# zhvng/open-musiclm

Measured on NVIDIA H100. Metric: coarse-stage training tokens/sec (positions fed to the transformer per optimiser step / step time), higher is better.
Workload: dtype bf16 (fp16 operands for the forward GEMMs on LayerNorm outputs x weights; fp32 accumulate)

## Files before the change

open-musiclm_b200/csrc/common.cuh:

```cuda
#pragma once
#include <cuda_runtime.h>
#include <cuda_bf16.h>
#include <cuda_fp16.h>
#include <cuda.h>
#include <stdint.h>
#include <stdio.h>

namespace omlm {

void set_last_error(const char* fmt, ...);
#define OMLM_CHECK_ARG(cond, ...)          \
  do {                                     \
    if (!(cond)) {                         \
      ::omlm::set_last_error(__VA_ARGS__); \
      return 1;                            \
    }                                      \
  } while (0)
#define OMLM_CUDA(expr)                                                                       \
  do {                                                                                        \
    cudaError_t _e = (expr);                                                                  \
    if (_e != cudaSuccess) {                                                                  \
      ::omlm::set_last_error("%s:%d %s -> %s", __FILE__, __LINE__, #expr, cudaGetErrorString(_e)); \
      return 1000 + static_cast<int>(_e);                                                     \
    }                                                                                         \
  } while (0)
#define OMLM_LAUNCH_CHECK() OMLM_CUDA(cudaGetLastError())

int make_tmap_bf16_2d(CUtensorMap* out, const void* gptr, uint64_t dim0, uint64_t dim1,
                      uint64_t pitch_bytes, uint32_t box0, uint32_t box1);

int make_tmap_2d(CUtensorMap* out, int elem_bytes, const void* gptr, uint64_t dim0, uint64_t dim1, uint64_t pitch_bytes,
                 uint32_t box0, uint32_t box1);

int make_tmap_bf16_3d(CUtensorMap* out, const void* gptr, uint64_t dim0, uint64_t dim1, uint64_t dim2,
                      uint64_t pitch1_bytes, uint64_t pitch2_bytes, uint32_t box0, uint32_t box1);

int num_sms();

template <typename... KArgs, typename... Args>
inline cudaError_t launch_k(void (*kern)(KArgs...), dim3 grid, dim3 block, size_t smem, cudaStream_t stream, Args&&... args) {
  cudaLaunchConfig_t cfg = {};
  cfg.gridDim = grid; cfg.blockDim = block; cfg.dynamicSmemBytes = smem; cfg.stream = stream;
  return cudaLaunchKernelEx(&cfg, kern, static_cast<KArgs>(args)...);
}
#define OMLM_KLAUNCH(kern, grid, block, smem, stream, ...)                                                   \
  do {                                                                                                       \
    cudaError_t _le = ::omlm::launch_k(kern, dim3(grid), dim3(block), smem, stream, __VA_ARGS__);            \
    if (_le != cudaSuccess) {                                                                                \
      ::omlm::set_last_error("%s:%d launch of %s -> %s", __FILE__, __LINE__, #kern, cudaGetErrorString(_le)); \
      return 1000 + static_cast<int>(_le);                                                                   \
    }                                                                                                        \
  } while (0)

__device__ __forceinline__ float warp_sum(float v) {
#pragma unroll
  for (int o = 16; o > 0; o >>= 1) v += __shfl_xor_sync(0xffffffffu, v, o);
  return v;
}
__device__ __forceinline__ float warp_max(float v) {
#pragma unroll
  for (int o = 16; o > 0; o >>= 1) v = fmaxf(v, __shfl_xor_sync(0xffffffffu, v, o));
  return v;
}
__device__ __forceinline__ uint32_t pack_bf16x2(float lo, float hi) {
  __nv_bfloat162 t = __floats2bfloat162_rn(lo, hi);
  return *reinterpret_cast<uint32_t*>(&t);
}
__device__ __forceinline__ float2 unpack_bf16x2(uint32_t v) {
  __nv_bfloat162 t = *reinterpret_cast<__nv_bfloat162*>(&v);
  return __bfloat1622float2(t);
}
__device__ __forceinline__ float bf16_round(float x) {
  return __bfloat162float(__float2bfloat16_rn(x));
}
enum : int { kFmtBF16 = 0, kFmtF32 = 1, kFmtF16 = 2 };
__device__ __forceinline__ uint32_t pack_f16x2(float lo, float hi) {
  uint32_t r;
  asm("cvt.rn.satfinite.f16x2.f32 %0, %1, %2;" : "=r"(r) : "f"(hi), "f"(lo));
  return r;
}
__device__ __forceinline__ float2 unpack_f16x2(uint32_t v) {
  __half2 t = *reinterpret_cast<__half2*>(&v);
  return __half22float2(t);
}
template <bool F16>
__device__ __forceinline__ uint32_t pack16x2(float lo, float hi) {
  if constexpr (F16) return pack_f16x2(lo, hi); else return pack_bf16x2(lo, hi);
}
template <bool F16>
__device__ __forceinline__ float2 unpack16x2(uint32_t v) {
  if constexpr (F16) return unpack_f16x2(v); else return unpack_bf16x2(v);
}

__device__ __forceinline__ float2 fma2(float2 a, float2 b, float2 c) { return make_float2(fmaf(a.x, b.x, c.x), fmaf(a.y, b.y, c.y)); }
__device__ __forceinline__ float2 mul2(float2 a, float2 b) { return make_float2(__fmul_rn(a.x, b.x), __fmul_rn(a.y, b.y)); }
__device__ __forceinline__ float2 add2(float2 a, float2 b) { return make_float2(__fadd_rn(a.x, b.x), __fadd_rn(a.y, b.y)); }
__device__ __forceinline__ float2 splat2(float v) { return make_float2(v, v); }
__device__ __forceinline__ float rcp_approx(float x) {
  float r;
  asm("rcp.approx.ftz.f32 %0, %1;" : "=f"(r) : "f"(x));
  return r;
}
__device__ __forceinline__ float ex2_approx(float x) {
  float r;
  asm("ex2.approx.ftz.f32 %0, %1;" : "=f"(r) : "f"(x));
// ... 52 lines not shown
```

open-musiclm_b200/csrc/gemm_ffn_up.cu:

```cuda
#include "common.cuh"
#include "ptx.cuh"
#include "../../include/omlm_b200.h"

namespace omlm {

constexpr int kFuBM = 128, kFuBN = 256, kFuBK = 64, kFuStages = 3, kFuRowsOut = 126;
constexpr int kFuA = kFuBM * kFuBK * 2, kFuB = kFuBN * kFuBK * 2, kFuStage = kFuA + kFuB;
constexpr int kFuUPitch = 528;
constexpr int kFuOffU = kFuStages * kFuStage;
constexpr int kFuOffBar = kFuOffU + kFuBM * kFuUPitch;
constexpr int kFuSmem = kFuOffBar + 256 + 1024;
constexpr int kFuThreads = 384;

template <bool F16>
__global__ void __launch_bounds__(kFuThreads, 1)
gemm_ffn_up_kernel(const __grid_constant__ CUtensorMap tmA, const __grid_constant__ CUtensorMap tmB,
                   __nv_bfloat16* __restrict__ u_out, __nv_bfloat16* __restrict__ h_out, float* __restrict__ rowsum,
                   const float* __restrict__ conv_w, int M, int Nseq, int K, int Fp) {
  extern __shared__ __align__(1024) uint8_t smem_raw[];
  uint8_t* smem = smem_raw + ((1024u - (smem_u32(smem_raw) & 1023u)) & 1023u);
  uint64_t* full_bar = reinterpret_cast<uint64_t*>(smem + kFuOffBar);
  uint64_t* empty_bar = full_bar + kFuStages;
  uint8_t* usm = smem + kFuOffU;

  const int wg = threadIdx.x >> 7, lane = threadIdx.x & 31;
  const int m_tiles = (M + kFuRowsOut - 1) / kFuRowsOut;
  const int n_tiles = (2 * Fp) / kFuBN;
  const int kb_total = (K + kFuBK - 1) / kFuBK;
  const int work_total = m_tiles * n_tiles;

  if (threadIdx.x == 0) {
    tma_prefetch_desc(&tmA); tma_prefetch_desc(&tmB);
    for (int i = 0; i < kFuStages; ++i) { mbar_init(&full_bar[i], 1); mbar_init(&empty_bar[i], 2); }
    fence_barrier_init();
  }
  __syncthreads();

  if (wg == 0) {
    asm volatile("setmaxnreg.dec.sync.aligned.u32 40;");
    if (threadIdx.x == 0) {
      int stage = 0; uint32_t phase = 0;
      for (int w = blockIdx.x; w < work_total; w += gridDim.x) {
        const int n_blk = w % n_tiles, m_blk = w / n_tiles;
        for (int kb = 0; kb < kb_total; ++kb) {
          mbar_wait(&empty_bar[stage], phase ^ 1);
          uint8_t* sa = smem + stage * kFuStage;
          mbar_expect_tx(&full_bar[stage], kFuStage);
          tma_load_2d(sa, &tmA, &full_bar[stage], kb * kFuBK, m_blk * kFuRowsOut - 2);
          tma_load_2d(sa + kFuA, &tmB, &full_bar[stage], kb * kFuBK, n_blk * kFuBN);
          if (++stage == kFuStages) { stage = 0; phase ^= 1; }
        }
      }
    }
  } else {
    asm volatile("setmaxnreg.inc.sync.aligned.u32 232;");
    const int cw = wg - 1;
    const int wq = (threadIdx.x >> 5) & 3, qr = lane >> 2, qc = lane & 3;
    const bool leader = (threadIdx.x & 127) == 0;
    const int et = threadIdx.x - 128;
    int stage = 0; uint32_t phase = 0;
    bool first = true;
    for (int w = blockIdx.x; w < work_total; w += gridDim.x) {
      const int n_blk = w % n_tiles, m_blk = w / n_tiles;
      float acc[kFuBN / 2];
#pragma unroll
      for (int i = 0; i < kFuBN / 2; ++i) acc[i] = 0.f;
      int prev = -1;
      for (int kb = 0; kb < kb_total; ++kb) {
        mbar_wait(&full_bar[stage], phase);
        const uint32_t sa = smem_u32(smem + stage * kFuStage) + cw * 8192, sb = smem_u32(smem + stage * kFuStage + kFuA);
        wgmma_fence();
#pragma unroll
        for (int k = 0; k < kFuBK / 16; ++k)
          Wgmma<kFuBN, F16>::template ss<0, 0>(acc, make_smem_desc(sa + k * 32, 16, 1024), make_smem_desc(sb + k * 32, 16, 1024),
                                               (kb > 0 || k > 0) ? 1u : 0u);
        wgmma_commit();
        wgmma_wait<1>();
        if (prev >= 0 && leader) mbar_arrive(&empty_bar[prev]);
        prev = stage;
        if (++stage == kFuStages) { stage = 0; phase ^= 1; }
      }
      wgmma_wait<0>();
      wgmma_reg_fence(acc);
      if (prev >= 0 && leader) mbar_arrive(&empty_bar[prev]);
      float2 wv[3][2], wg2[3][2];
      {
        const float4* wp = reinterpret_cast<const float4*>(conv_w + static_cast<long>(n_blk * kFuBN + lane * 4) * 3);
        const float4* gp = reinterpret_cast<const float4*>(conv_w + static_cast<long>(n_blk * kFuBN + 128 + lane * 4) * 3);
        const float4 a0 = __ldg(wp), a1 = __ldg(wp + 1), a2 = __ldg(wp + 2);
        const float4 b0 = __ldg(gp), b1 = __ldg(gp + 1), b2 = __ldg(gp + 2);
        const float fa[12] = {a0.x, a0.y, a0.z, a0.w, a1.x, a1.y, a1.z, a1.w, a2.x, a2.y, a2.z, a2.w};
        const float fb[12] = {b0.x, b0.y, b0.z, b0.w, b1.x, b1.y, b1.z, b1.w, b2.x, b2.y, b2.z, b2.w};
#pragma unroll
        for (int k = 0; k < 3; ++k)
#pragma unroll
          for (int q = 0; q < 2; ++q) {
            wv[k][q] = make_float2(fa[(2 * q) * 3 + k], fa[(2 * q + 1) * 3 + k]);
            wg2[k][q] = make_float2(fb[(2 * q) * 3 + k], fb[(2 * q + 1) * 3 + k]);
          }
      }
      if (!first) asm volatile("bar.sync 2, 256;" ::: "memory");
      first = false;
#pragma unroll
      for (int hr = 0; hr < 2; ++hr) {
        uint8_t* urow = usm + (cw * 64 + wq * 16 + qr + hr * 8) * kFuUPitch + qc * 4;
#pragma unroll
        for (int i = 0; i < kFuBN / 8; ++i)
          *reinterpret_cast<uint32_t*>(urow + i * 16) = pack16x2<F16>(acc[4 * i + 2 * hr], acc[4 * i + 2 * hr + 1]);
      }
      asm volatile("bar.sync 2, 256;" ::: "memory");
      {
        const int ew = et >> 5;
        const int t0 = 2 + ew * 16;
        const long grow0 = static_cast<long>(m_blk) * kFuRowsOut - 2 + t0;
        const int nrows = min(min(16, kFuBM - t0), static_cast<int>(min(static_cast<long>(16), M - grow0)));
        int pos = static_cast<int>(grow0 % Nseq);
        const uint8_t* rp = usm + t0 * kFuUPitch;
        float2 xv1[2], xg1[2], xv2[2], xg2[2];
        {
          const uint2 a = *reinterpret_cast<const uint2*>(rp - kFuUPitch + lane * 8);
          const uint2 g = *reinterpret_cast<const uint2*>(rp - kFuUPitch + 256 + lane * 8);
          xv1[0] = unpack16x2<F16>(a.x); xv1[1] = unpack16x2<F16>(a.y); xg1[0] = unpack16x2<F16>(g.x); xg1[1] = unpack16x2<F16>(g.y);
        }
        {
          const uint2 a = *reinterpret_cast<const uint2*>(rp - 2 * kFuUPitch + lane * 8);
          const uint2 g = *reinterpret_cast<const uint2*>(rp - 2 * kFuUPitch + 256 + lane * 8);
          xv2[0] = unpack16x2<F16>(a.x); xv2[1] = unpack16x2<F16>(a.y); xg2[0] = unpack16x2<F16>(g.x); xg2[1] = unpack16x2<F16>(g.y);
        }
        if (pos == 1) { xv2[0] = xv2[1] = xg2[0] = xg2[1] = make_float2(0.f, 0.f); }
        float st[32];
        __nv_bfloat16* ug = u_out + grow0 * (2L * Fp) + n_blk * kFuBN + lane * 8;
        __nv_bfloat16* hg = h_out + grow0 * static_cast<long>(Fp) + n_blk * 128 + lane * 4;
#pragma unroll
        for (int r = 0; r < 16; ++r) {
          float s1 = 0.f, s2 = 0.f;
          if (r < nrows) {
            const uint8_t* rr = rp + r * kFuUPitch;
            *reinterpret_cast<uint4*>(ug + static_cast<long>(r) * (2L * Fp)) = *reinterpret_cast<const uint4*>(rr + lane * 16);
            const uint2 a = *reinterpret_cast<const uint2*>(rr + lane * 8);
            const uint2 g = *reinterpret_cast<const uint2*>(rr + 256 + lane * 8);
            const float2 xv0[2] = {unpack16x2<F16>(a.x), unpack16x2<F16>(a.y)}, xg0[2] = {unpack16x2<F16>(g.x), unpack16x2<F16>(g.y)};
            if (pos == 0) {
              const float2 z = make_float2(0.f, 0.f);
              xv1[0] = xv1[1] = xg1[0] = xg1[1] = z;
              xv2[0] = xv2[1] = xg2[0] = xg2[1] = z;
            }
            float2 h[2], sq = make_float2(0.f, 0.f), sm = sq;
#pragma unroll
            for (int q = 0; q < 2; ++q) {
              const float2 yv = fma2(wv[0][q], xv2[q], fma2(wv[1][q], xv1[q], mul2(wv[2][q], xv0[q])));
              const float2 yg = fma2(wg2[0][q], xg2[q], fma2(wg2[1][q], xg1[q], mul2(wg2[2][q], xg0[q])));
              h[q] = mul2(gelu_erf2(yg), yv);
              sm = add2(sm, h[q]);
              sq = fma2(h[q], h[q], sq);
              xv2[q] = xv1[q]; xv1[q] = xv0[q];
              xg2[q] = xg1[q]; xg1[q] = xg0[q];
            }
            s1 = sm.x + sm.y; s2 = sq.x + sq.y;
            *reinterpret_cast<uint2*>(hg + static_cast<long>(r) * Fp) = make_uint2(pack16x2<F16>(h[0].x, h[0].y), pack16x2<F16>(h[1].x, h[1].y));
            if (++pos == Nseq) pos = 0;
          }
          st[2 * r] = s1;
          st[2 * r + 1] = s2;
        }
#pragma unroll
        for (int off = 16; off >= 1; off >>= 1) {
          const bool hi = (lane & off) != 0;
#pragma unroll
          for (int i = 0; i < off; ++i) {
            const float send = hi ? st[i] : st[i + off];
            const float keep = hi ? st[i + off] : st[i];
            st[i] = keep + __shfl_xor_sync(0xffffffffu, send, off);
          }
        }
        if ((lane >> 1) < nrows) rowsum[(grow0 + (lane >> 1)) * (2L * n_tiles) + 2 * n_blk + (lane & 1)] = st[0];
      }
    }
  }
}

}

extern "C" int omlm_gemm_ffn_up(const void* xn, const void* w1_packed, const float* conv_w_packed, void* u_out, void* h_out,
                                float* rowsum, int M, int Nseq, int K, int Fp, int act_f16, int max_ctas, void* stream) {
  using namespace omlm;
  OMLM_CHECK_ARG(M > 0 && Nseq > 0 && K > 0 && K % 8 == 0 && Fp > 0 && Fp % 128 == 0, "gemm_ffn_up: bad shape M=%d K=%d Fp=%d", M, K, Fp);
  CUtensorMap tmA, tmB;
  int rc = make_tmap_bf16_2d(&tmA, xn, static_cast<uint64_t>(K), static_cast<uint64_t>(M), static_cast<uint64_t>(K) * 2, 64, kFuBM);
  if (rc) return rc;
  rc = make_tmap_bf16_2d(&tmB, w1_packed, static_cast<uint64_t>(K), static_cast<uint64_t>(2 * Fp), static_cast<uint64_t>(K) * 2, 64, kFuBN);
  if (rc) return rc;
  static bool configured = false;
  if (!configured) {
    OMLM_CUDA(cudaFuncSetAttribute(gemm_ffn_up_kernel<false>, cudaFuncAttributeMaxDynamicSharedMemorySize, kFuSmem));
    OMLM_CUDA(cudaFuncSetAttribute(gemm_ffn_up_kernel<true>, cudaFuncAttributeMaxDynamicSharedMemorySize, kFuSmem));
    configured = true;
  }
  const int m_tiles = (M + kFuRowsOut - 1) / kFuRowsOut, n_tiles = (2 * Fp) / kFuBN;
  int grid = num_sms();
  if (max_ctas > 0 && max_ctas < grid) grid = max_ctas;
  if (m_tiles * n_tiles < grid) grid = m_tiles * n_tiles;
  auto kern = act_f16 ? gemm_ffn_up_kernel<true> : gemm_ffn_up_kernel<false>;
  OMLM_KLAUNCH((kern), grid, kFuThreads, kFuSmem, reinterpret_cast<cudaStream_t>(stream), 
      tmA, tmB, reinterpret_cast<__nv_bfloat16*>(u_out), reinterpret_cast<__nv_bfloat16*>(h_out), rowsum, conv_w_packed, M,
      Nseq, K, Fp);
  OMLM_LAUNCH_CHECK();
  return 0;
}
```

open-musiclm_b200/csrc/gemm_tc.cu:

```cuda
#include "common.cuh"
#include "ptx.cuh"
#include "../../include/omlm_b200.h"
#include <stdlib.h>
#include <string.h>
#include <algorithm>

namespace omlm {

constexpr int BM = 128;
constexpr int BK = 64;
constexpr int kGemmThreads = 384;

struct EpiParams {
  void* out;
  const float* addend;
  long ldo;
  long ldadd;
  float alpha;
  int out_f32;
  int atomic;
  long split_stride;
  int vec_ok;
  int staged;
  int row_split;
  int row_valid;
  int n_valid;
  const float* rs_gamma;
  const uint8_t* rs_keep;
  float2* rs_part;
  float rs_keep_scale;
  int rs_parts;
};

__device__ __forceinline__ float bf16lo(uint32_t v) { return __uint_as_float(v << 16); }
__device__ __forceinline__ float bf16hi(uint32_t v) { return __uint_as_float(v & 0xffff0000u); }

template <int BN>
struct GemmSmem {
  static constexpr int kABytes = BM * BK * 2;
  static constexpr int kBBytes = BN * BK * 2;
  static constexpr int kStageBytes = kABytes + kBBytes;
  static constexpr int kMaxStages = 8;
};

constexpr int kEpiBoxes = 4;
constexpr int kBoxBytes = 64 * 128;
constexpr int kStagingBytes = 2 * kEpiBoxes * kBoxBytes;

__device__ __forceinline__ void wg_bar_sync(int cw) { asm volatile("bar.sync %0, 128;" ::"r"(1 + cw) : "memory"); }

template <bool F32>
__device__ __forceinline__ uint32_t box_offset(int r, int g, int qc) {
  const int chunk = F32 ? 2 * g + (qc >> 1) : g;
  return r * 128 + ((chunk ^ (r & 7)) << 4) + (F32 ? 8 * (qc & 1) : 4 * qc);
}

__device__ __forceinline__ void load_box(const CUtensorMap* tm, uint8_t* box, uint64_t* bar, int col, int row) {
  mbar_expect_tx(bar, kBoxBytes);
  tma_load_2d(box, tm, bar, col, row);
}

template <int BN, bool RS, bool F32>
__device__ __forceinline__ void epilogue_staged(float (&acc)[BN / 2], const EpiParams& ep, const CUtensorMap* tmO,
                                                const CUtensorMap* tmE, uint8_t* ring, uint64_t* ebar, uint32_t& seq,
                                                uint32_t& ephase, int live, int n_blk, int row0, int M, int N, int cw,
                                                bool leader) {
  constexpr int kCols = F32 ? 32 : 64, kGroups = kCols / 8, kBoxesPerTile = BN / kCols;
  constexpr int kBatch = RS ? 4 : kGroups;
  const bool with_e = RS || ep.addend != nullptr;
  const int lane = threadIdx.x & 31, wq = (threadIdx.x >> 5) & 3, qr = lane >> 2, qc = lane & 3;
  float rs1[2][2] = {{0.f, 0.f}, {0.f, 0.f}}, rs2[2][2] = {{0.f, 0.f}, {0.f, 0.f}};
#pragma unroll
  for (int b = 0; b < kBoxesPerTile; ++b) {
    if (b >= live) break;
    const uint32_t slot = seq % kEpiBoxes;
    uint8_t* box = ring + slot * kBoxBytes;
    if (with_e) {
      mbar_wait(&ebar[slot], (ephase >> slot) & 1u);
      ephase ^= 1u << slot;
    } else {
      if (leader) tma_store_wait_read<kEpiBoxes - 1>();
      wg_bar_sync(cw);
    }
#pragma unroll
    for (int g0 = 0; g0 < kGroups; g0 += kBatch) {
      float2 gam[kBatch];
      uint32_t keep[2][kBatch];
      if constexpr (RS) {
#pragma unroll
        for (int j = 0; j < kBatch; ++j) {
          const int col = n_blk * BN + b * kCols + 8 * (g0 + j) + 2 * qc;
          gam[j] = __ldg(reinterpret_cast<const float2*>(ep.rs_gamma + col));
#pragma unroll
          for (int hr = 0; hr < 2; ++hr) {
            const int row = row0 + wq * 16 + qr + hr * 8;
            keep[hr][j] = (row < M && ep.rs_keep != nullptr) ? ep.rs_keep[static_cast<long>(row) * (N >> 3) + (col >> 3)] : 0xffu;
          }
        }
      }
#pragma unroll
      for (int j = 0; j < kBatch; ++j) {
        const int i = b * kGroups + g0 + j;
#pragma unroll
        for (int hr = 0; hr < 2; ++hr) {
          const int r = wq * 16 + qr + hr * 8;
          uint8_t* p = box + box_offset<F32>(r, g0 + j, qc);
          float v0 = __fmul_rn(acc[4 * i + 2 * hr], ep.alpha), v1 = __fmul_rn(acc[4 * i + 2 * hr + 1], ep.alpha);
          if constexpr (RS) {
            const uint32_t kb = keep[hr][j], hv = *reinterpret_cast<const uint32_t*>(p);
            const int col = n_blk * BN + 8 * i + 2 * qc;
            const int hf = (8 * i) / (BN / 2);
            rs1[hr][hf] = fmaf(gam[j].x, ((kb >> (col & 7)) & 1u) ? v0 : 0.f, rs1[hr][hf]);
            rs1[hr][hf] = fmaf(gam[j].y, ((kb >> ((col + 1) & 7)) & 1u) ? v1 : 0.f, rs1[hr][hf]);
            rs2[hr][hf] = fmaf(v0, bf16lo(hv), rs2[hr][hf]);
            rs2[hr][hf] = fmaf(v1, bf16hi(hv), rs2[hr][hf]);
          }
          if constexpr (F32) {
            if (ep.addend != nullptr) { const float2 a = *reinterpret_cast<const float2*>(p); v0 += a.x; v1 += a.y; }
            *reinterpret_cast<float2*>(p) = make_float2(v0, v1);
          } else {
            *reinterpret_cast<uint32_t*>(p) = pack_bf16x2(v0, v1);
          }
        }
      }
    }
    fence_proxy_async();
    wg_bar_sync(cw);
    if (leader) {
      tma_store_2d(tmO, box, n_blk * BN + b * kCols, row0);
      tma_store_commit();
      if (with_e && b >= 1 && b - 1 + kEpiBoxes < live) {
        const uint32_t s = (seq - 1) % kEpiBoxes;
        tma_store_wait_read<1>();
        load_box(tmE, ring + s * kBoxBytes, &ebar[s], n_blk * BN + (b - 1 + kEpiBoxes) * kCols, row0);
      }
    }
    ++seq;
  }
  if constexpr (RS) {
#pragma unroll
    for (int hr = 0; hr < 2; ++hr)
#pragma unroll
      for (int hf = 0; hf < 2; ++hf) {
        float a1 = rs1[hr][hf], a2 = rs2[hr][hf];
        a1 += __shfl_xor_sync(0xffffffffu, a1, 1); a1 += __shfl_xor_sync(0xffffffffu, a1, 2);
        a2 += __shfl_xor_sync(0xffffffffu, a2, 1); a2 += __shfl_xor_sync(0xffffffffu, a2, 2);
        const int row = row0 + wq * 16 + qr + hr * 8;
        if (qc == 0 && row < M) ep.rs_part[static_cast<long>(row) * ep.rs_parts + 2 * n_blk + hf] = make_float2(a1 * ep.rs_keep_scale, a2);
      }
  }
}

template <int BN, int A_MN, int B_MN, bool F16, bool RS = false>
__global__ void __launch_bounds__(kGemmThreads, 1)
gemm_bf16_kernel(const __grid_constant__ CUtensorMap tmA, const __grid_constant__ CUtensorMap tmB,
                 const __grid_constant__ CUtensorMap tmO, const __grid_constant__ CUtensorMap tmE,
                 const EpiParams ep, const int M, const int N, const int K, const int splits, const int kStages) {
  using S = GemmSmem<BN>;
  extern __shared__ uint8_t smem_raw[];
  uint8_t* smem = smem_raw + ((1024u - (smem_u32(smem_raw) & 1023u)) & 1023u);
  uint8_t* staging = smem + kStages * S::kStageBytes;
  uint64_t* full_bar = reinterpret_cast<uint64_t*>(staging + (ep.staged ? kStagingBytes : 0));
  uint64_t* empty_bar = full_bar + S::kMaxStages;
  uint64_t* epi_bar = empty_bar + S::kMaxStages;

  const int wg = threadIdx.x >> 7;
  const int lane = threadIdx.x & 31;

  const int m_tiles = (M + BM - 1) / BM;
  const int n_tiles = (N + BN - 1) / BN;
  const int kb_total = (K + BK - 1) / BK;
  const int kb_per_split = (kb_total + splits - 1) / splits;
  const int tiles_total = m_tiles * n_tiles;
  const int work_total = tiles_total * splits;

  if (threadIdx.x == 0) {
    tma_prefetch_desc(&tmA);
    tma_prefetch_desc(&tmB);
    for (int i = 0; i < kStages; ++i) {
      mbar_init(&full_bar[i], 1);
      mbar_init(&empty_bar[i], 2);
    }
    if (ep.staged) {
      tma_prefetch_desc(&tmO);
      for (int i = 0; i < 2 * kEpiBoxes; ++i) mbar_init(&epi_bar[i], 1);
    }
    fence_barrier_init();
  }
  __syncthreads();

  if (wg == 0) {
    asm volatile("setmaxnreg.dec.sync.aligned.u32 40;");
    if (threadIdx.x == 0) {
      int stage = 0;
      uint32_t phase = 0;
      for (int w = blockIdx.x; w < work_total; w += gridDim.x) {
        const int split = w / tiles_total;
        const int tile = w - split * tiles_total;
        const int n_blk = tile % n_tiles, m_blk = tile / n_tiles;
        const int kb0 = split * kb_per_split;
        const int kb1 = min(kb_total, kb0 + kb_per_split);
        for (int kb = kb0; kb < kb1; ++kb) {
          mbar_wait(&empty_bar[stage], phase ^ 1);
          uint8_t* sa = smem + stage * S::kStageBytes;
          uint8_t* sb = sa + S::kABytes;
          mbar_expect_tx(&full_bar[stage], S::kStageBytes);
          if (A_MN == 0) {
            tma_load_2d(sa, &tmA, &full_bar[stage], kb * BK, m_blk * BM);
          } else {
#pragma unroll
            for (int c = 0; c < BM / 64; ++c)
              tma_load_2d(sa + c * 8192, &tmA, &full_bar[stage], m_blk * BM + c * 64, kb * BK);
          }
          if (B_MN == 0) {
            tma_load_2d(sb, &tmB, &full_bar[stage], kb * BK, n_blk * BN);
          } else {
#pragma unroll
            for (int c = 0; c < BN / 64; ++c)
              tma_load_2d(sb + c * 8192, &tmB, &full_bar[stage], n_blk * BN + c * 64, kb * BK);
          }
          if (++stage == kStages) { stage = 0; phase ^= 1; }
        }
      }
    }
    return;
  }

  asm volatile("setmaxnreg.inc.sync.aligned.u32 232;");
  const int cw = wg - 1;
  const int wq = (threadIdx.x >> 5) & 3;
  const int qr = lane >> 2, qc = lane & 3;
  const bool leader = (threadIdx.x & 127) == 0;
  uint8_t* ring = staging + cw * kEpiBoxes * kBoxBytes;
  uint64_t* ebar = epi_bar + cw * kEpiBoxes;
  const bool with_e = ep.staged && (RS || ep.addend != nullptr);
  const int box_cols = (RS || !ep.out_f32) ? 64 : 32;
  uint32_t seq = 0, ephase = 0;
  int stage = 0;
  uint32_t phase = 0;
  for (int w = blockIdx.x; w < work_total; w += gridDim.x) {
    const int split = w / tiles_total;
    const int tile = w - split * tiles_total;
    const int n_blk = tile % n_tiles, m_blk = tile / n_tiles;
    const int kb0 = split * kb_per_split;
    const int kb1 = min(kb_total, kb0 + kb_per_split);
    const int row0 = m_blk * BM + cw * 64;
    const int live = row0 < M ? max(0, min(BN / box_cols, (ep.n_valid - n_blk * BN + box_cols - 1) / box_cols)) : 0;
    if (with_e && leader) {
      tma_store_wait_read<0>();
      for (int j = 0; j < min(kEpiBoxes, live); ++j) {
        const uint32_t s = (seq + j) % kEpiBoxes;
        load_box(&tmE, ring + s * kBoxBytes, &ebar[s], n_blk * BN + j * box_cols, row0);
      }
    }
    float acc[BN / 2];
#pragma unroll
    for (int i = 0; i < BN / 2; ++i) acc[i] = 0.f;
    int prev = -1;
    for (int kb = kb0; kb < kb1; ++kb) {
      mbar_wait(&full_bar[stage], phase);
      const uint32_t sa = smem_u32(smem + stage * S::kStageBytes) + cw * 8192;
      const uint32_t sb = smem_u32(smem + stage * S::kStageBytes + S::kABytes);
      wgmma_fence();
#pragma unroll
      for (int k = 0; k < BK / 16; ++k) {
        const uint64_t ad = A_MN ? make_smem_desc(sa + k * 2048, 8192, 1024) : make_smem_desc(sa + k * 32, 16, 1024);
        const uint64_t bd = B_MN ? make_smem_desc(sb + k * 2048, 8192, 1024) : make_smem_desc(sb + k * 32, 16, 1024);
        const uint32_t accum = (kb > kb0 || k > 0) ? 1u : 0u;
        Wgmma<BN, F16>::template ss<A_MN, B_MN>(acc, ad, bd, accum);
      }
      wgmma_commit();
      wgmma_wait<1>();
      if (prev >= 0 && leader) mbar_arrive(&empty_bar[prev]);
      prev = stage;
      if (++stage == kStages) { stage = 0; phase ^= 1; }
    }
    wgmma_wait<0>();
    wgmma_reg_fence(acc);
    if (prev >= 0 && leader) mbar_arrive(&empty_bar[prev]);

    if constexpr (RS) {
      epilogue_staged<BN, true, false>(acc, ep, &tmO, &tmE, ring, ebar, seq, ephase, live, n_blk, row0, M, N, cw, leader);
    } else if (ep.staged) {
      if (ep.out_f32) epilogue_staged<BN, false, true>(acc, ep, &tmO, &tmE, ring, ebar, seq, ephase, live, n_blk, row0, M, N, cw, leader);
      else epilogue_staged<BN, false, false>(acc, ep, &tmO, &tmE, ring, ebar, seq, ephase, live, n_blk, row0, M, N, cw, leader);
    } else {
      long orow[2], arow[2];
      bool row_ok[2];
  #pragma unroll
      for (int hr = 0; hr < 2; ++hr) {
        int row = m_blk * BM + cw * 64 + wq * 16 + qr + hr * 8;
        row_ok[hr] = row < M;
        if (ep.row_split > 0) {
          const int half = row / ep.row_split, r = row - half * ep.row_split;
          row_ok[hr] = row_ok[hr] && r < ep.row_valid;
          row = half * ep.row_valid + r;
        } else if (ep.row_split < 0) {
          const int w256 = row & 255, ch = ((row >> 8) << 7) + (w256 & 127);
          row_ok[hr] = row_ok[hr] && ch < ep.row_valid;
          row = (w256 >> 7) * ep.row_valid + ch;
        }
        orow[hr] = static_cast<long>(row) * ep.ldo;
        arow[hr] = static_cast<long>(row) * ep.ldadd;
      }
      constexpr int kEpiBatch = 8;
  #pragma unroll
      for (int i0 = 0; i0 < BN / 8; i0 += kEpiBatch) {
        float2 add[2][kEpiBatch];
  #pragma unroll
        for (int j = 0; j < kEpiBatch; ++j) {
          const int col = n_blk * BN + 8 * (i0 + j) + 2 * qc;
          const bool c0_ok = col < ep.n_valid, c1_ok = col + 1 < ep.n_valid;
  #pragma unroll
          for (int hr = 0; hr < 2; ++hr) {
            add[hr][j] = make_float2(0.f, 0.f);
            if (!row_ok[hr] || !c0_ok) continue;
            if (ep.addend != nullptr) {
              const float* ap = ep.addend + arow[hr] + col;
              if (c1_ok && ep.vec_ok) add[hr][j] = *reinterpret_cast<const float2*>(ap);
              else { add[hr][j].x = ap[0]; if (c1_ok) add[hr][j].y = ap[1]; }
            }
          }
        }
  #pragma unroll
        for (int j = 0; j < kEpiBatch; ++j) {
          const int i = i0 + j;
          const int col = n_blk * BN + 8 * i + 2 * qc;
          if (col >= ep.n_valid) continue;
          const bool pair = col + 1 < ep.n_valid && ep.vec_ok;
  #pragma unroll
          for (int hr = 0; hr < 2; ++hr) {
            if (!row_ok[hr]) continue;
            float v0 = __fmul_rn(acc[4 * i + 2 * hr], ep.alpha), v1 = __fmul_rn(acc[4 * i + 2 * hr + 1], ep.alpha);
            if (ep.addend != nullptr) { v0 += add[hr][j].x; v1 += add[hr][j].y; }
            if (ep.atomic) {
              float* op = reinterpret_cast<float*>(ep.out) + orow[hr] + col;
              if (pair) asm volatile("red.global.add.v2.f32 [%0], {%1, %2};" ::"l"(op), "f"(v0), "f"(v1) : "memory");
              else { atomicAdd(op, v0); if (col + 1 < ep.n_valid) atomicAdd(op + 1, v1); }
            } else if (ep.out_f32) {
              float* op = reinterpret_cast<float*>(ep.out) + split * ep.split_stride + orow[hr] + col;
              if (pair) *reinterpret_cast<float2*>(op) = make_float2(v0, v1);
              else { op[0] = v0; if (col + 1 < ep.n_valid) op[1] = v1; }
            } else {
              __nv_bfloat16* op = reinterpret_cast<__nv_bfloat16*>(ep.out) + orow[hr] + col;
              if (pair) *reinterpret_cast<uint32_t*>(op) = pack_bf16x2(v0, v1);
              else { op[0] = __float2bfloat16_rn(v0); if (col + 1 < ep.n_valid) op[1] = __float2bfloat16_rn(v1); }
            }
          }
        }
      }
    }
  }
  if (ep.staged && leader) tma_store_wait_all();
}

constexpr int kMaxDynSmem = 232448;
constexpr int kBarrierBytes = 256;

template <int BN, int A_MN, int B_MN, bool RS = false>
static int launch_gemm(const CUtensorMap& tmA, const CUtensorMap& tmB, const CUtensorMap& tmO, const CUtensorMap& tmE,
                       const EpiParams& ep, int M, int N, int K, int splits, int max_ctas, int f16, cudaStream_t stream) {
  using S = GemmSmem<BN>;
  auto kern = f16 ? gemm_bf16_kernel<BN, A_MN, B_MN, true, RS> : gemm_bf16_kernel<BN, A_MN, B_MN, false, RS>;
  const int staging = ep.staged ? kStagingBytes : 0;
  int stages = (kMaxDynSmem - 1024 - kBarrierBytes - staging) / S::kStageBytes;
  if (stages > 6) stages = 6;
  const int smem_bytes = stages * S::kStageBytes + staging + kBarrierBytes + 1024;
  static bool configured[2] = {false, false};
  if (!configured[f16]) {
    OMLM_CUDA(cudaFuncSetAttribute(kern, cudaFuncAttributeMaxDynamicSharedMemorySize, kMaxDynSmem));
    configured[f16] = true;
  }
  const int m_tiles = (M + BM - 1) / BM, n_tiles = (N + BN - 1) / BN;
  const int work = m_tiles * n_tiles * splits;
  int grid = num_sms();
  if (max_ctas > 0 && max_ctas < grid) grid = max_ctas;
  if (work < grid) grid = work;
  OMLM_KLAUNCH((kern), grid, kGemmThreads, smem_bytes, stream, tmA, tmB, tmO, tmE, ep, M, N, K, splits, stages);
  OMLM_LAUNCH_CHECK();
  return 0;
}

}

namespace omlm {
struct RowStatArgs { const void* hn; long ldhn; const void* keep_bits; const float* gamma; float keep_scale; float* part; int parts; };
}

static int gemm16_impl(const void* A, int a_f16, int a_mn_major, long lda, const void* B, int b_f16, int b_mn_major,
                       long ldb, int M, int N, int K, void* out, int out_f32, long ldo,
                       const float* addend, long ldadd, float alpha, int splits,
                       int row_split, int row_valid, int n_valid, int block_n, int max_ctas,
                       void* stream_, const omlm::RowStatArgs* rs, long split_stride = 0) {
  using namespace omlm;
  cudaStream_t stream = reinterpret_cast<cudaStream_t>(stream_);
  OMLM_CHECK_ARG(M > 0 && N > 0 && K > 0, "gemm: empty problem %d x %d x %d", M, N, K);
  OMLM_CHECK_ARG(block_n == 128 || block_n == 256, "gemm: block_n must be 128 or 256");
  OMLM_CHECK_ARG(splits >= 1, "gemm: splits must be >= 1");
  OMLM_CHECK_ARG((a_f16 != 0) == (b_f16 != 0), "gemm: both operands must have the same 16-bit format (one wgmma takes one operand format)");
  OMLM_CHECK_ARG(splits == 1 || (out_f32 && addend == nullptr), "gemm: split-K needs fp32 atomic output and no addend");
  OMLM_CHECK_ARG(split_stride == 0 || (out_f32 && addend == nullptr && rs == nullptr), "gemm: partial slices need fp32 output");
  if (n_valid <= 0 || n_valid > N) n_valid = N;
  const bool accumulate = splits > 1 && split_stride == 0;
  {
    const int kb_total = (K + BK - 1) / BK;
    if (splits > kb_total) splits = kb_total;
    const int per = (kb_total + splits - 1) / splits;
    splits = (kb_total + per - 1) / per;
  }
  CUtensorMap tmA, tmB;
  int rc;
  if (a_mn_major == 0) rc = make_tmap_bf16_2d(&tmA, A, (uint64_t)K, (uint64_t)M, (uint64_t)lda * 2, 64, BM);
  else                 rc = make_tmap_bf16_2d(&tmA, A, (uint64_t)M, (uint64_t)K, (uint64_t)lda * 2, 64, 64);
  if (rc) return rc;
  if (b_mn_major == 0) rc = make_tmap_bf16_2d(&tmB, B, (uint64_t)K, (uint64_t)N, (uint64_t)ldb * 2, 64, block_n);
  else                 rc = make_tmap_bf16_2d(&tmB, B, (uint64_t)N, (uint64_t)K, (uint64_t)ldb * 2, 64, 64);
  if (rc) return rc;
  EpiParams ep;
  ep.out = out; ep.addend = addend; ep.ldo = ldo; ep.ldadd = ldadd; ep.alpha = alpha;
  ep.out_f32 = out_f32; ep.atomic = accumulate ? 1 : 0; ep.split_stride = split_stride;
  const long esz = out_f32 ? 4 : 2;
  ep.vec_ok = ((ldo * esz) % 16 == 0) && ((reinterpret_cast<uintptr_t>(out) & 15) == 0) &&
              (addend == nullptr || ((ldadd * 4) % 16 == 0 && (reinterpret_cast<uintptr_t>(addend) & 15) == 0));
  ep.row_split = row_split; ep.row_valid = row_valid; ep.n_valid = n_valid;
  ep.rs_gamma = nullptr; ep.rs_keep = nullptr; ep.rs_part = nullptr; ep.rs_keep_scale = 1.f; ep.rs_parts = 0;
  ep.staged = !ep.atomic && split_stride == 0 && row_split == 0 && ep.vec_ok && (addend == nullptr || out_f32) &&
              (n_valid * esz) % 16 == 0;
  CUtensorMap tmO, tmE;
  memset(&tmO, 0, sizeof(tmO));
  memset(&tmE, 0, sizeof(tmE));
  if (ep.staged) {
    rc = make_tmap_2d(&tmO, static_cast<int>(esz), out, (uint64_t)n_valid, (uint64_t)M, (uint64_t)(ldo * esz), out_f32 ? 32 : 64, 64);
    if (rc == 0 && addend != nullptr) rc = make_tmap_2d(&tmE, 4, addend, (uint64_t)n_valid, (uint64_t)M, (uint64_t)(ldadd * 4), 32, 64);
// ... 122 lines not shown
```

open-musiclm_b200/csrc/ptx.cuh:

```cuda
#pragma once
#include <cuda_runtime.h>
#include <cuda_bf16.h>
#include <cuda.h>
#include <stdint.h>

namespace omlm {

__device__ __forceinline__ uint32_t smem_u32(const void* p) {
  return static_cast<uint32_t>(__cvta_generic_to_shared(p));
}
__device__ __forceinline__ uint32_t lane_id() { return threadIdx.x & 31; }

__device__ __forceinline__ bool elect_one() {
  uint32_t pred;
  asm volatile(
      "{\n\t.reg .pred p;\n\t"
      "elect.sync _|p, 0xffffffff;\n\t"
      "selp.u32 %0, 1, 0, p;\n\t}"
      : "=r"(pred));
  return pred != 0;
}

__device__ __forceinline__ void mbar_init(uint64_t* bar, uint32_t count) {
  asm volatile("mbarrier.init.shared::cta.b64 [%0], %1;" ::"r"(smem_u32(bar)), "r"(count));
}
__device__ __forceinline__ void fence_barrier_init() {
  asm volatile("fence.mbarrier_init.release.cluster;" ::: "memory");
}
__device__ __forceinline__ void fence_proxy_async() {
  asm volatile("fence.proxy.async.shared::cta;" ::: "memory");
}
__device__ __forceinline__ void mbar_expect_tx(uint64_t* bar, uint32_t bytes) {
  asm volatile("mbarrier.arrive.expect_tx.shared::cta.b64 _, [%0], %1;" ::"r"(smem_u32(bar)),
               "r"(bytes)
               : "memory");
}
__device__ __forceinline__ void mbar_arrive(uint64_t* bar) {
  asm volatile("mbarrier.arrive.shared::cta.b64 _, [%0];" ::"r"(smem_u32(bar)) : "memory");
}
__device__ __forceinline__ void mbar_wait(uint64_t* bar, uint32_t parity) {
  asm volatile(
      "{\n\t.reg .pred p;\n\t"
      "WAIT_LOOP:\n\t"
      "mbarrier.try_wait.parity.shared::cta.b64 p, [%0], %1;\n\t"
      "@p bra DONE;\n\t"
      "bra WAIT_LOOP;\n\t"
      "DONE:\n\t}"
      ::"r"(smem_u32(bar)), "r"(parity)
      : "memory");
}

__device__ __forceinline__ void tma_prefetch_desc(const CUtensorMap* m) {
  asm volatile("prefetch.tensormap [%0];" ::"l"(reinterpret_cast<uint64_t>(m)) : "memory");
}
__device__ __forceinline__ void tma_load_2d(void* smem_dst, const CUtensorMap* m, uint64_t* bar,
                                            int32_t c0, int32_t c1) {
  asm volatile(
      "cp.async.bulk.tensor.2d.shared::cluster.global.mbarrier::complete_tx::bytes"
      " [%0], [%1, {%3, %4}], [%2];"
      ::"r"(smem_u32(smem_dst)), "l"(reinterpret_cast<uint64_t>(m)), "r"(smem_u32(bar)), "r"(c0),
      "r"(c1)
      : "memory");
}
__device__ __forceinline__ void tma_store_2d(const CUtensorMap* m, const void* smem_src, int32_t c0,
                                             int32_t c1) {
  asm volatile("cp.async.bulk.tensor.2d.global.shared::cta.bulk_group [%0, {%2, %3}], [%1];"
               ::"l"(reinterpret_cast<uint64_t>(m)), "r"(smem_u32(smem_src)), "r"(c0), "r"(c1)
               : "memory");
}
__device__ __forceinline__ void tma_store_3d(const CUtensorMap* m, const void* smem_src, int32_t c0, int32_t c1,
                                             int32_t c2) {
  asm volatile("cp.async.bulk.tensor.3d.global.shared::cta.bulk_group [%0, {%2, %3, %4}], [%1];"
               ::"l"(reinterpret_cast<uint64_t>(m)), "r"(smem_u32(smem_src)), "r"(c0), "r"(c1), "r"(c2)
               : "memory");
}
__device__ __forceinline__ void tma_store_commit() {
  asm volatile("cp.async.bulk.commit_group;" ::: "memory");
}
__device__ __forceinline__ void tma_store_wait_all() {
  asm volatile("cp.async.bulk.wait_group 0;" ::: "memory");
}
template <int N>
__device__ __forceinline__ void tma_store_wait_read() {
  asm volatile("cp.async.bulk.wait_group.read %0;" ::"n"(N) : "memory");
}

__device__ __forceinline__ void wgmma_fence() { asm volatile("wgmma.fence.sync.aligned;" ::: "memory"); }
__device__ __forceinline__ void wgmma_commit() { asm volatile("wgmma.commit_group.sync.aligned;" ::: "memory"); }
template <int N>
__device__ __forceinline__ void wgmma_wait() { asm volatile("wgmma.wait_group.sync.aligned %0;" ::"n"(N) : "memory"); }
template <int R>
__device__ __forceinline__ void wgmma_reg_fence(float (&d)[R]) {
#pragma unroll
  for (int i = 0; i < R; ++i) asm volatile("" : "+f"(d[i])::"memory");
}

__device__ __forceinline__ uint64_t make_smem_desc(uint32_t smem_addr, uint32_t lbo_bytes,
                                                   uint32_t sbo_bytes) {
  uint64_t d = 0;
  d |= static_cast<uint64_t>((smem_addr & 0x3FFFF) >> 4);
  d |= static_cast<uint64_t>((lbo_bytes >> 4) & 0x3FFF) << 16;
  d |= static_cast<uint64_t>((sbo_bytes >> 4) & 0x3FFF) << 32;
  d |= static_cast<uint64_t>(1) << 62;
  return d;
}

template <int N, bool F16> struct Wgmma;
template <> struct Wgmma<64, false> {
  template <int TA, int TB>
  static __device__ __forceinline__ void ss(float (&d)[32], uint64_t a, uint64_t b, uint32_t scale_d) {
    asm volatile(
        "{\n.reg .pred p;\nsetp.ne.b32 p, %34, 0;\n"
        "wgmma.mma_async.sync.aligned.m64n64k16.f32.bf16.bf16 {%0,%1,%2,%3,%4,%5,%6,%7,%8,%9,%10,%11,%12,%13,%14,%15,%16,%17,%18,%19,%20,%21,%22,%23,%24,%25,%26,%27,%28,%29,%30,%31}, %32, %33, p, 1, 1, %35, %36;\n}\n"
        : "+f"(d[0]), "+f"(d[1]), "+f"(d[2]), "+f"(d[3]), "+f"(d[4]), "+f"(d[5]), "+f"(d[6]), "+f"(d[7]), "+f"(d[8]), "+f"(d[9]), "+f"(d[10]), "+f"(d[11]), "+f"(d[12]), "+f"(d[13]), "+f"(d[14]), "+f"(d[15]), "+f"(d[16]), "+f"(d[17]), "+f"(d[18]), "+f"(d[19]), "+f"(d[20]), "+f"(d[21]), "+f"(d[22]), "+f"(d[23]), "+f"(d[24]), "+f"(d[25]), "+f"(d[26]), "+f"(d[27]), "+f"(d[28]), "+f"(d[29]), "+f"(d[30]), "+f"(d[31])
// ... 72 lines not shown
```

Measured before the change: 801,700.

## Multicast FFN-up weight tiles across 2-CTA clusters and shrink epilogue staging for long K

The FFN-up GEMM now launches as 2-CTA clusters. Each CTA loads half of the shared B (weight) tile and multicasts it to both CTAs, so each weight tile is fetched from global/L2 once per pair of M tiles. Empty barriers count arrivals from both CTAs, and cluster syncs bracket the kernel. Separately, the generic GEMM makes the epilogue staging ring size a template parameter and uses 2 boxes instead of 4 for BN=256 long-K staged GEMMs, freeing shared memory for more pipeline stages. The cost is cross-CTA coupling, since the two CTAs must stay in lockstep, and possible tail imbalance from the odd m_tiles padding.

```diff
diff --git a/open-musiclm_b200/csrc/common.cuh b/open-musiclm_b200/csrc/common.cuh
--- a/open-musiclm_b200/csrc/common.cuh
+++ b/open-musiclm_b200/csrc/common.cuh
@@ -38,19 +38,46 @@
 int num_sms();
 
 template <typename... KArgs, typename... Args>
-inline cudaError_t launch_k(void (*kern)(KArgs...), dim3 grid, dim3 block, size_t smem, cudaStream_t stream, Args&&... args) {
+inline cudaError_t launch_kc(void (*kern)(KArgs...), dim3 grid, dim3 block, size_t smem, cudaStream_t stream, int cluster,
+                             Args&&... args) {
   cudaLaunchConfig_t cfg = {};
   cfg.gridDim = grid; cfg.blockDim = block; cfg.dynamicSmemBytes = smem; cfg.stream = stream;
+  cudaLaunchAttribute attr[1];
+  if (cluster > 1) {
+    attr[0].id = cudaLaunchAttributeClusterDimension;
+    attr[0].val.clusterDim.x = cluster; attr[0].val.clusterDim.y = 1; attr[0].val.clusterDim.z = 1;
+    cfg.attrs = attr; cfg.numAttrs = 1;
+  }
   return cudaLaunchKernelEx(&cfg, kern, static_cast<KArgs>(args)...);
 }
-#define OMLM_KLAUNCH(kern, grid, block, smem, stream, ...)                                                   \
+template <typename... KArgs, typename... Args>
+inline cudaError_t launch_k(void (*kern)(KArgs...), dim3 grid, dim3 block, size_t smem, cudaStream_t stream, Args&&... args) {
+  return launch_kc(kern, grid, block, smem, stream, 1, static_cast<Args&&>(args)...);
+}
+template <typename... KArgs>
+inline int max_active_clusters(void (*kern)(KArgs...), int block, size_t smem, int cluster) {
+  cudaLaunchConfig_t cfg = {};
+  cfg.gridDim = dim3(cluster); cfg.blockDim = dim3(block); cfg.dynamicSmemBytes = smem;
+  cudaLaunchAttribute attr[1];
+  attr[0].id = cudaLaunchAttributeClusterDimension;
+  attr[0].val.clusterDim.x = cluster; attr[0].val.clusterDim.y = 1; attr[0].val.clusterDim.z = 1;
+  cfg.attrs = attr; cfg.numAttrs = 1;
+  int n = 0;
+  if (cudaOccupancyMaxActiveClusters(&n, kern, &cfg) != cudaSuccess) {
+    (void)cudaGetLastError();
+    return 0;
+  }
+  return n;
+}
+#define OMLM_KLAUNCH_CLUSTER(kern, grid, block, smem, stream, cluster, ...)                                  \
   do {                                                                                                       \
-    cudaError_t _le = ::omlm::launch_k(kern, dim3(grid), dim3(block), smem, stream, __VA_ARGS__);            \
+    cudaError_t _le = ::omlm::launch_kc(kern, dim3(grid), dim3(block), smem, stream, cluster, __VA_ARGS__);  \
     if (_le != cudaSuccess) {                                                                                \
       ::omlm::set_last_error("%s:%d launch of %s -> %s", __FILE__, __LINE__, #kern, cudaGetErrorString(_le)); \
       return 1000 + static_cast<int>(_le);                                                                   \
     }                                                                                                        \
   } while (0)
+#define OMLM_KLAUNCH(kern, grid, block, smem, stream, ...) OMLM_KLAUNCH_CLUSTER(kern, grid, block, smem, stream, 1, __VA_ARGS__)
 
 __device__ __forceinline__ float warp_sum(float v) {
 #pragma unroll
diff --git a/open-musiclm_b200/csrc/gemm_ffn_up.cu b/open-musiclm_b200/csrc/gemm_ffn_up.cu
--- a/open-musiclm_b200/csrc/gemm_ffn_up.cu
+++ b/open-musiclm_b200/csrc/gemm_ffn_up.cu
@@ -1,6 +1,7 @@
 #include "common.cuh"
 #include "ptx.cuh"
 #include "../../include/omlm_b200.h"
+#include <algorithm>
 
 namespace omlm {
 
@@ -11,6 +12,15 @@
 constexpr int kFuOffBar = kFuOffU + kFuBM * kFuUPitch;
 constexpr int kFuSmem = kFuOffBar + 256 + 1024;
 constexpr int kFuThreads = 384;
+
+__device__ __forceinline__ void release_stage(uint64_t* bar, int cs) {
+  if (cs == 1) {
+    mbar_arrive(bar);
+  } else {
+    mbar_arrive_cluster(bar, 0);
+    mbar_arrive_cluster(bar, 1);
+  }
+}
 
 template <bool F16>
 __global__ void __launch_bounds__(kFuThreads, 1)
@@ -24,30 +34,36 @@
   uint8_t* usm = smem + kFuOffU;
 
   const int wg = threadIdx.x >> 7, lane = threadIdx.x & 31;
+  const int cs = static_cast<int>(cluster_nctarank()), crank = static_cast<int>(cluster_ctarank());
   const int m_tiles = (M + kFuRowsOut - 1) / kFuRowsOut;
   const int n_tiles = (2 * Fp) / kFuBN;
   const int kb_total = (K + kFuBK - 1) / kFuBK;
-  const int work_total = m_tiles * n_tiles;
+  const int work_total = (m_tiles + cs - 1) / cs * n_tiles;
+  const int w_first = blockIdx.x / cs, w_step = gridDim.x / cs;
 
   if (threadIdx.x == 0) {
     tma_prefetch_desc(&tmA); tma_prefetch_desc(&tmB);
-    for (int i = 0; i < kFuStages; ++i) { mbar_init(&full_bar[i], 1); mbar_init(&empty_bar[i], 2); }
+    for (int i = 0; i < kFuStages; ++i) { mbar_init(&full_bar[i], 1); mbar_init(&empty_bar[i], 2 * cs); }
     fence_barrier_init();
   }
-  __syncthreads();
+  if (cs > 1) cluster_sync(); else __syncthreads();
 
   if (wg == 0) {
     asm volatile("setmaxnreg.dec.sync.aligned.u32 40;");
     if (threadIdx.x == 0) {
       int stage = 0; uint32_t phase = 0;
-      for (int w = blockIdx.x; w < work_total; w += gridDim.x) {
-        const int n_blk = w % n_tiles, m_blk = w / n_tiles;
+      for (int w = w_first; w < work_total; w += w_step) {
+        const int n_blk = w % n_tiles, m_blk = w / n_tiles * cs + crank;
         for (int kb = 0; kb < kb_total; ++kb) {
           mbar_wait(&empty_bar[stage], phase ^ 1);
           uint8_t* sa = smem + stage * kFuStage;
           mbar_expect_tx(&full_bar[stage], kFuStage);
           tma_load_2d(sa, &tmA, &full_bar[stage], kb * kFuBK, m_blk * kFuRowsOut - 2);
-          tma_load_2d(sa + kFuA, &tmB, &full_bar[stage], kb * kFuBK, n_blk * kFuBN);
+          if (cs == 1)
+            tma_load_2d(sa + kFuA, &tmB, &full_bar[stage], kb * kFuBK, n_blk * kFuBN);
+          else
+            tma_load_2d_multicast(sa + kFuA + crank * (kFuBN / 2) * 128, &tmB, &full_bar[stage], kb * kFuBK,
+                                  n_blk * kFuBN + crank * (kFuBN / 2), 0x3);
           if (++stage == kFuStages) { stage = 0; phase ^= 1; }
         }
       }
@@ -60,8 +76,8 @@
     const int et = threadIdx.x - 128;
     int stage = 0; uint32_t phase = 0;
     bool first = true;
-    for (int w = blockIdx.x; w < work_total; w += gridDim.x) {
-      const int n_blk = w % n_tiles, m_blk = w / n_tiles;
+    for (int w = w_first; w < work_total; w += w_step) {
+      const int n_blk = w % n_tiles, m_blk = w / n_tiles * cs + crank;
       float acc[kFuBN / 2];
 #pragma unroll
       for (int i = 0; i < kFuBN / 2; ++i) acc[i] = 0.f;
@@ -76,13 +92,13 @@
                                                (kb > 0 || k > 0) ? 1u : 0u);
         wgmma_commit();
         wgmma_wait<1>();
-        if (prev >= 0 && leader) mbar_arrive(&empty_bar[prev]);
+        if (prev >= 0 && leader) release_stage(&empty_bar[prev], cs);
         prev = stage;
         if (++stage == kFuStages) { stage = 0; phase ^= 1; }
       }
       wgmma_wait<0>();
       wgmma_reg_fence(acc);
-      if (prev >= 0 && leader) mbar_arrive(&empty_bar[prev]);
+      if (prev >= 0 && leader) release_stage(&empty_bar[prev], cs);
       float2 wv[3][2], wg2[3][2];
       {
         const float4* wp = reinterpret_cast<const float4*>(conv_w + static_cast<long>(n_blk * kFuBN + lane * 4) * 3);
@@ -177,6 +193,7 @@
       }
     }
   }
+  if (cs > 1) cluster_sync();
 }
 
 }
@@ -188,7 +205,10 @@
   CUtensorMap tmA, tmB;
   int rc = make_tmap_bf16_2d(&tmA, xn, static_cast<uint64_t>(K), static_cast<uint64_t>(M), static_cast<uint64_t>(K) * 2, 64, kFuBM);
   if (rc) return rc;
-  rc = make_tmap_bf16_2d(&tmB, w1_packed, static_cast<uint64_t>(K), static_cast<uint64_t>(2 * Fp), static_cast<uint64_t>(K) * 2, 64, kFuBN);
+  const int m_tiles = (M + kFuRowsOut - 1) / kFuRowsOut, n_tiles = (2 * Fp) / kFuBN;
+  const int cluster = max_ctas == 1 ? 1 : 2;
+  rc = make_tmap_bf16_2d(&tmB, w1_packed, static_cast<uint64_t>(K), static_cast<uint64_t>(2 * Fp), static_cast<uint64_t>(K) * 2, 64,
+                         kFuBN / cluster);
   if (rc) return rc;
   static bool configured = false;
   if (!configured) {
@@ -196,12 +216,21 @@
     OMLM_CUDA(cudaFuncSetAttribute(gemm_ffn_up_kernel<true>, cudaFuncAttributeMaxDynamicSharedMemorySize, kFuSmem));
     configured = true;
   }
-  const int m_tiles = (M + kFuRowsOut - 1) / kFuRowsOut, n_tiles = (2 * Fp) / kFuBN;
-  int grid = num_sms();
-  if (max_ctas > 0 && max_ctas < grid) grid = max_ctas;
-  if (m_tiles * n_tiles < grid) grid = m_tiles * n_tiles;
   auto kern = act_f16 ? gemm_ffn_up_kernel<true> : gemm_ffn_up_kernel<false>;
-  OMLM_KLAUNCH((kern), grid, kFuThreads, kFuSmem, reinterpret_cast<cudaStream_t>(stream), 
+  int grid;
+  if (cluster == 1) {
+    grid = num_sms();
+    if (max_ctas > 0 && max_ctas < grid) grid = max_ctas;
+    if (m_tiles * n_tiles < grid) grid = m_tiles * n_tiles;
+  } else {
+    static int fit = -1;
+    if (fit < 0) fit = max_active_clusters(kern, kFuThreads, kFuSmem, 2);
+    OMLM_CHECK_ARG(fit > 0, "gemm_ffn_up: no 2-CTA cluster of %d bytes of shared memory per CTA fits on this device", kFuSmem);
+    int clusters = std::min(fit, (m_tiles + 1) / 2 * n_tiles);
+    if (max_ctas > 0) clusters = std::min(clusters, max_ctas / 2);
+    grid = 2 * clusters;
+  }
+  OMLM_KLAUNCH_CLUSTER((kern), grid, kFuThreads, kFuSmem, reinterpret_cast<cudaStream_t>(stream), cluster,
       tmA, tmB, reinterpret_cast<__nv_bfloat16*>(u_out), reinterpret_cast<__nv_bfloat16*>(h_out), rowsum, conv_w_packed, M,
       Nseq, K, Fp);
   OMLM_LAUNCH_CHECK();
diff --git a/open-musiclm_b200/csrc/gemm_tc.cu b/open-musiclm_b200/csrc/gemm_tc.cu
--- a/open-musiclm_b200/csrc/gemm_tc.cu
+++ b/open-musiclm_b200/csrc/gemm_tc.cu
@@ -43,9 +43,8 @@
   static constexpr int kMaxStages = 8;
 };
 
-constexpr int kEpiBoxes = 4;
 constexpr int kBoxBytes = 64 * 128;
-constexpr int kStagingBytes = 2 * kEpiBoxes * kBoxBytes;
+constexpr int kLongKBlocks = 32;
 
 __device__ __forceinline__ void wg_bar_sync(int cw) { asm volatile("bar.sync %0, 128;" ::"r"(1 + cw) : "memory"); }
 
@@ -60,7 +59,7 @@
   tma_load_2d(box, tm, bar, col, row);
 }
 
-template <int BN, bool RS, bool F32>
+template <int BN, bool RS, bool F32, int NB>
 __device__ __forceinline__ void epilogue_staged(float (&acc)[BN / 2], const EpiParams& ep, const CUtensorMap* tmO,
                                                 const CUtensorMap* tmE, uint8_t* ring, uint64_t* ebar, uint32_t& seq,
                                                 uint32_t& ephase, int live, int n_blk, int row0, int M, int N, int cw,
@@ -73,13 +72,13 @@
 #pragma unroll
   for (int b = 0; b < kBoxesPerTile; ++b) {
     if (b >= live) break;
-    const uint32_t slot = seq % kEpiBoxes;
+    const uint32_t slot = seq % NB;
     uint8_t* box = ring + slot * kBoxBytes;
     if (with_e) {
       mbar_wait(&ebar[slot], (ephase >> slot) & 1u);
       ephase ^= 1u << slot;
     } else {
-      if (leader) tma_store_wait_read<kEpiBoxes - 1>();
+      if (leader) tma_store_wait_read<NB - 1>();
       wg_bar_sync(cw);
     }
 #pragma unroll
@@ -129,10 +128,10 @@
     if (leader) {
       tma_store_2d(tmO, box, n_blk * BN + b * kCols, row0);
       tma_store_commit();
-      if (with_e && b >= 1 && b - 1 + kEpiBoxes < live) {
-        const uint32_t s = (seq - 1) % kEpiBoxes;
+      if (with_e && b >= 1 && b - 1 + NB < live) {
+        const uint32_t s = (seq - 1) % NB;
         tma_store_wait_read<1>();
-        load_box(tmE, ring + s * kBoxBytes, &ebar[s], n_blk * BN + (b - 1 + kEpiBoxes) * kCols, row0);
+        load_box(tmE, ring + s * kBoxBytes, &ebar[s], n_blk * BN + (b - 1 + NB) * kCols, row0);
       }
     }
     ++seq;
@@ -151,7 +150,7 @@
   }
 }
 
-template <int BN, int A_MN, int B_MN, bool F16, bool RS = false>
+template <int BN, int A_MN, int B_MN, bool F16, bool RS, int NB>
 __global__ void __launch_bounds__(kGemmThreads, 1)
 gemm_bf16_kernel(const __grid_constant__ CUtensorMap tmA, const __grid_constant__ CUtensorMap tmB,
                  const __grid_constant__ CUtensorMap tmO, const __grid_constant__ CUtensorMap tmE,
@@ -160,7 +159,7 @@
   extern __shared__ uint8_t smem_raw[];
   uint8_t* smem = smem_raw + ((1024u - (smem_u32(smem_raw) & 1023u)) & 1023u);
   uint8_t* staging = smem + kStages * S::kStageBytes;
-  uint64_t* full_bar = reinterpret_cast<uint64_t*>(staging + (ep.staged ? kStagingBytes : 0));
+  uint64_t* full_bar = reinterpret_cast<uint64_t*>(staging + (ep.staged ? 2 * NB * kBoxBytes : 0));
   uint64_t* empty_bar = full_bar + S::kMaxStages;
   uint64_t* epi_bar = empty_bar + S::kMaxStages;
 
@@ -183,7 +182,7 @@
     }
     if (ep.staged) {
       tma_prefetch_desc(&tmO);
-      for (int i = 0; i < 2 * kEpiBoxes; ++i) mbar_init(&epi_bar[i], 1);
+      for (int i = 0; i < 2 * NB; ++i) mbar_init(&epi_bar[i], 1);
     }
     fence_barrier_init();
   }
@@ -231,8 +230,8 @@
   const int wq = (threadIdx.x >> 5) & 3;
   const int qr = lane >> 2, qc = lane & 3;
   const bool leader = (threadIdx.x & 127) == 0;
-  uint8_t* ring = staging + cw * kEpiBoxes * kBoxBytes;
-  uint64_t* ebar = epi_bar + cw * kEpiBoxes;
+  uint8_t* ring = staging + cw * NB * kBoxBytes;
+  uint64_t* ebar = epi_bar + cw * NB;
   const bool with_e = ep.staged && (RS || ep.addend != nullptr);
   const int box_cols = (RS || !ep.out_f32) ? 64 : 32;
   uint32_t seq = 0, ephase = 0;
@@ -248,8 +247,8 @@
     const int live = row0 < M ? max(0, min(BN / box_cols, (ep.n_valid - n_blk * BN + box_cols - 1) / box_cols)) : 0;
     if (with_e && leader) {
       tma_store_wait_read<0>();
-      for (int j = 0; j < min(kEpiBoxes, live); ++j) {
-        const uint32_t s = (seq + j) % kEpiBoxes;
+      for (int j = 0; j < min(NB, live); ++j) {
+        const uint32_t s = (seq + j) % NB;
         load_box(&tmE, ring + s * kBoxBytes, &ebar[s], n_blk * BN + j * box_cols, row0);
       }
     }
@@ -280,10 +279,10 @@
     if (prev >= 0 && leader) mbar_arrive(&empty_bar[prev]);
 
     if constexpr (RS) {
-      epilogue_staged<BN, true, false>(acc, ep, &tmO, &tmE, ring, ebar, seq, ephase, live, n_blk, row0, M, N, cw, leader);
+      epilogue_staged<BN, true, false, NB>(acc, ep, &tmO, &tmE, ring, ebar, seq, ephase, live, n_blk, row0, M, N, cw, leader);
     } else if (ep.staged) {
-      if (ep.out_f32) epilogue_staged<BN, false, true>(acc, ep, &tmO, &tmE, ring, ebar, seq, ephase, live, n_blk, row0, M, N, cw, leader);
-      else epilogue_staged<BN, false, false>(acc, ep, &tmO, &tmE, ring, ebar, seq, ephase, live, n_blk, row0, M, N, cw, leader);
+      if (ep.out_f32) epilogue_staged<BN, false, true, NB>(acc, ep, &tmO, &tmE, ring, ebar, seq, ephase, live, n_blk, row0, M, N, cw, leader);
+      else epilogue_staged<BN, false, false, NB>(acc, ep, &tmO, &tmE, ring, ebar, seq, ephase, live, n_blk, row0, M, N, cw, leader);
     } else {
       long orow[2], arow[2];
       bool row_ok[2];
@@ -357,12 +356,12 @@
 constexpr int kMaxDynSmem = 232448;
 constexpr int kBarrierBytes = 256;
 
-template <int BN, int A_MN, int B_MN, bool RS = false>
-static int launch_gemm(const CUtensorMap& tmA, const CUtensorMap& tmB, const CUtensorMap& tmO, const CUtensorMap& tmE,
-                       const EpiParams& ep, int M, int N, int K, int splits, int max_ctas, int f16, cudaStream_t stream) {
+template <int BN, int A_MN, int B_MN, bool RS, int NB>
+static int launch_gemm_nb(const CUtensorMap& tmA, const CUtensorMap& tmB, const CUtensorMap& tmO, const CUtensorMap& tmE,
+                          const EpiParams& ep, int M, int N, int K, int splits, int max_ctas, int f16, cudaStream_t stream) {
   using S = GemmSmem<BN>;
-  auto kern = f16 ? gemm_bf16_kernel<BN, A_MN, B_MN, true, RS> : gemm_bf16_kernel<BN, A_MN, B_MN, false, RS>;
-  const int staging = ep.staged ? kStagingBytes : 0;
+  auto kern = f16 ? gemm_bf16_kernel<BN, A_MN, B_MN, true, RS, NB> : gemm_bf16_kernel<BN, A_MN, B_MN, false, RS, NB>;
+  const int staging = ep.staged ? 2 * NB * kBoxBytes : 0;
   int stages = (kMaxDynSmem - 1024 - kBarrierBytes - staging) / S::kStageBytes;
   if (stages > 6) stages = 6;
   const int smem_bytes = stages * S::kStageBytes + staging + kBarrierBytes + 1024;
@@ -379,6 +378,16 @@
   OMLM_KLAUNCH((kern), grid, kGemmThreads, smem_bytes, stream, tmA, tmB, tmO, tmE, ep, M, N, K, splits, stages);
   OMLM_LAUNCH_CHECK();
   return 0;
+}
+
+template <int BN, int A_MN, int B_MN, bool RS = false>
+static int launch_gemm(const CUtensorMap& tmA, const CUtensorMap& tmB, const CUtensorMap& tmO, const CUtensorMap& tmE,
+                       const EpiParams& ep, int M, int N, int K, int splits, int max_ctas, int f16, cudaStream_t stream) {
+  if constexpr (BN == 256 && !RS) {
+    if (ep.staged && (K + BK - 1) / BK >= kLongKBlocks)
+      return launch_gemm_nb<BN, A_MN, B_MN, RS, 2>(tmA, tmB, tmO, tmE, ep, M, N, K, splits, max_ctas, f16, stream);
+  }
+  return launch_gemm_nb<BN, A_MN, B_MN, RS, 4>(tmA, tmB, tmO, tmE, ep, M, N, K, splits, max_ctas, f16, stream);
 }
 
 }
diff --git a/open-musiclm_b200/csrc/ptx.cuh b/open-musiclm_b200/csrc/ptx.cuh
--- a/open-musiclm_b200/csrc/ptx.cuh
+++ b/open-musiclm_b200/csrc/ptx.cuh
@@ -50,6 +50,28 @@
       : "memory");
 }
 
+__device__ __forceinline__ uint32_t cluster_ctarank() {
+  uint32_t r;
+  asm volatile("mov.u32 %0, %%cluster_ctarank;" : "=r"(r));
+  return r;
+}
+__device__ __forceinline__ uint32_t cluster_nctarank() {
+  uint32_t r;
+  asm volatile("mov.u32 %0, %%cluster_nctarank;" : "=r"(r));
+  return r;
+}
+__device__ __forceinline__ void cluster_sync() {
+  asm volatile("barrier.cluster.arrive.release;\n\tbarrier.cluster.wait.acquire;" ::: "memory");
+}
+__device__ __forceinline__ void mbar_arrive_cluster(uint64_t* bar, uint32_t rank) {
+  asm volatile(
+      "{\n\t.reg .b32 ra;\n\t"
+      "mapa.shared::cluster.u32 ra, %0, %1;\n\t"
+      "mbarrier.arrive.shared::cluster.b64 _, [ra];\n\t}"
+      ::"r"(smem_u32(bar)), "r"(rank)
+      : "memory");
+}
+
 __device__ __forceinline__ void tma_prefetch_desc(const CUtensorMap* m) {
   asm volatile("prefetch.tensormap [%0];" ::"l"(reinterpret_cast<uint64_t>(m)) : "memory");
 }
@@ -60,6 +82,14 @@
       " [%0], [%1, {%3, %4}], [%2];"
       ::"r"(smem_u32(smem_dst)), "l"(reinterpret_cast<uint64_t>(m)), "r"(smem_u32(bar)), "r"(c0),
       "r"(c1)
+      : "memory");
+}
+__device__ __forceinline__ void tma_load_2d_multicast(void* smem_dst, const CUtensorMap* m, uint64_t* bar, int32_t c0,
+                                                      int32_t c1, uint16_t cta_mask) {
+  asm volatile(
+      "cp.async.bulk.tensor.2d.shared::cluster.global.mbarrier::complete_tx::bytes.multicast::cluster"
+      " [%0], [%1, {%3, %4}], [%2], %5;"
+      ::"r"(smem_u32(smem_dst)), "l"(reinterpret_cast<uint64_t>(m)), "r"(smem_u32(bar)), "r"(c0), "r"(c1), "h"(cta_mask)
       : "memory");
 }
 __device__ __forceinline__ void tma_store_2d(const CUtensorMap* m, const void* smem_src, int32_t c0,
```

After: 807,100 (median of 6 runs). No clear change (+0.7%).
